# bjkomer/pyratslam

Measured on AMD Instinct MI355X. Metric: pose-cell steps/sec (64×64×36) + template-compares/sec at 1/2/4/8 GPU, higher is better.
Workload: dtype u8; 1 GPU; configs[1]: 64x64x36 pose-cell grid + 1000 stored 64x32 u8 templates per GPU; a step matches 10 batches of 1024 queries resident in HBM; templates_per_gpu=1000, templates_total=1000, queries_per_batch=1024, parallelism=library sharded over 1 GPU(s), none; pose cells replicated

## Files before the change

### pyratslam_amd/csrc/view_templates.hip

```cpp
#include <hip/hip_runtime.h>
#include <rccl/rccl.h>

#include <algorithm>
#include <climits>
#include <cstdint>
#include <cstdio>
#include <cstdlib>
#include <cstring>
#include <memory>
#include <vector>

#include "rs_common.h"
#include "vt_plan.h"

namespace {

constexpr int FAST_M = 8;
constexpr unsigned long long NO_KEY = ~0ull;

__device__ inline unsigned long long wave_min_u64(unsigned long long v) {
#pragma unroll
    for (int off = 32; off > 0; off >>= 1) {
        const unsigned long long o = __shfl_xor(v, off);
        v = o < v ? o : v;
// ... 821 lines not shown
                                       wave, cg, lane, failed, ids, tk, v0);
    if (threadIdx.x == 0 && tk.takes && failed == tk.last) *ctr = 0u;
    if constexpr (!MATRIX) {
        if (out.host) {
            __shared__ int s_last;
            asm volatile("s_waitcnt vmcnt(0)" ::: "memory");
            __syncthreads();
            if (threadIdx.x == 0) {
                __builtin_amdgcn_fence(__ATOMIC_RELEASE, "agent");
                s_last = __hip_atomic_fetch_add(out.done, 1u, __ATOMIC_RELAXED, __HIP_MEMORY_SCOPE_AGENT) ==
                         gridDim.x - 1;
                if (s_last) __builtin_amdgcn_fence(__ATOMIC_ACQUIRE, "agent");
            }
            __syncthreads();
            if (s_last) {
                for (int i = threadIdx.x; i < nq; i += blockDim.x) {
                    const unsigned long long k =
                        __hip_atomic_load(out.best + i, __ATOMIC_RELAXED, __HIP_MEMORY_SCOPE_AGENT);
                    __hip_atomic_store(out.best + i, ~0ull, __ATOMIC_RELAXED, __HIP_MEMORY_SCOPE_AGENT);
                    __hip_atomic_store(out.host + i, k, __ATOMIC_RELAXED, __HIP_MEMORY_SCOPE_SYSTEM);
                }
                if (threadIdx.x == 0) __hip_atomic_store(out.done, 0u, __ATOMIC_RELAXED, __HIP_MEMORY_SCOPE_AGENT);
            }
        }
    }
    VT_STAMP(6);
}

constexpr int PF_WAVES = 4;
#ifndef VT_PF_TPW
#define VT_PF_TPW (VT_PF_UNITS == 1 ? 8 / (VT_PF_CGS) : 1)
#endif
constexpr int PF_TPW = VT_PF_TPW;
#ifndef VT_PF_CPS
#define VT_PF_CPS (VT_PF_TPW >= 4 ? 1 : 2)
#endif
constexpr int PF_CPS = VT_PF_CPS;
#ifndef VT_PF_GRID_CAP
#define VT_PF_GRID_CAP 4096
#endif
constexpr int PF_NB = 4;
constexpr int PF_QW4 = PF_NU * PF_CGS * PL_NO * 2;
constexpr uint32_t PF_NONE = (1u << 26) - 1u;

__device__ __forceinline__ uint32_t wave_min_u32_dpp(uint32_t v) {
    v = min(v, (uint32_t)__builtin_amdgcn_update_dpp((int)v, (int)v, 0xB1, 0xF, 0xF, false));
    v = min(v, (uint32_t)__builtin_amdgcn_update_dpp((int)v, (int)v, 0x4E, 0xF, 0xF, false));
    v = min(v, (uint32_t)__builtin_amdgcn_update_dpp((int)v, (int)v, 0x141, 0xF, 0xF, false));
    v = min(v, (uint32_t)__builtin_amdgcn_update_dpp((int)v, (int)v, 0x140, 0xF, 0xF, false));
    return min(min((uint32_t)__builtin_amdgcn_readlane((int)v, 0), (uint32_t)__builtin_amdgcn_readlane((int)v, 16)),
               min((uint32_t)__builtin_amdgcn_readlane((int)v, 32), (uint32_t)__builtin_amdgcn_readlane((int)v, 48)));
}

__global__ __launch_bounds__(64 * PF_WAVES) __attribute__((amdgpu_waves_per_eu(4)))
void vt_prefilter_kernel(const uint4* __restrict__ planes, int ntb,
                                                                    int64_t count,
                                                                    const uint4* __restrict__ qc4,
                                                                    const uint32_t* __restrict__ qsj, int nq,
                                                                    uint32_t* __restrict__ minlb,
                                                                    uint32_t* __restrict__ second) {
    constexpr int M = FAST_M, NU = 64 / 4, S0 = M - 3;
    static_assert(PF_CGS % PF_CPS == 0 && PF_CGS >= 1 && PF_CGS <= PL_CG, "whole steps of column groups, of the unit");
    static_assert(PF_NU * PF_CGS * 32 * 255 < (int)PF_NONE, "a bound and a lane fit one word");
    __shared__ uint4 s_q[PF_NB][PF_NU][PF_CGS][PL_NO][2];
    __shared__ uint32_t s_qs[PF_NB][PF_NU][16];
    const int wave = __builtin_amdgcn_readfirstlane(threadIdx.x >> 6), lane = threadIdx.x & 63;
    const int tb0 = (blockIdx.x * PF_WAVES + wave) * PF_TPW;
    const bool live = tb0 < ntb;
    uint32_t P[PF_TPW][PF_NU][PF_CGS][8], ts[PF_TPW][PF_NU];
    bool valid[PF_TPW];
#pragma unroll
    for (int t = 0; t < PF_TPW; ++t) {
        const int tbc = min(tb0 + t, ntb - 1);
        valid[t] = tb0 + t < ntb && (int64_t)(tb0 + t) * 64 + lane < count;
#pragma unroll
        for (int u = 0; u < PF_NU; ++u) {
            ts[t][u] = 0u;
#pragma unroll
            for (int cg = 0; cg < PF_CGS; ++cg) {
                const uint4* src = planes + ((size_t)(tbc * PL_CG + cg) * NU + pf_unit(u)) * 128 + lane;
                const uint4 a = src[0], b = src[64];
                uint32_t(&p)[8] = P[t][u][cg];
                p[0] = a.x; p[1] = a.y; p[2] = a.z; p[3] = a.w;
                p[4] = b.x; p[5] = b.y; p[6] = b.z; p[7] = b.w;
#pragma unroll
                for (int k = 0; k < 8; ++k) ts[t][u] += (uint32_t)__builtin_popcount(p[k]) << k;
            }
        }
    }
    for (int q0 = blockIdx.y * PF_NB; q0 < nq; q0 += gridDim.y * PF_NB) {
        const int nb = min(PF_NB, nq - q0);
        __syncthreads();
        for (int i = threadIdx.x; i < nb * PF_QW4; i += blockDim.x) {
            const int qq = i / PF_QW4, r = i - qq * PF_QW4;
            const int u = r / (PF_CGS * PL_NO * 2), r2 = r - u * (PF_CGS * PL_NO * 2);
            const int cg = r2 / (PL_NO * 2), w = r2 - cg * (PL_NO * 2);
            (&s_q[0][0][0][0][0])[i] = qc_unit(qc4 + (size_t)(q0 + qq) * QC_Q4, cg,
                                               4 * pf_unit(u) - (M - 1) - S0 + (w >> 1), w & 1);
        }
        if ((int)threadIdx.x < nb * PF_NU * 16)
            (&s_qs[0][0][0])[threadIdx.x] = qsj[(size_t)q0 * PF_NU * 16 + threadIdx.x];
        __syncthreads();
        if (!live) continue;
#pragma unroll 1
        for (int qq = 0; qq < nb; ++qq) {
            uint32_t m[PF_TPW];
#pragma unroll
            for (int t = 0; t < PF_TPW; ++t) m[t] = 0xFFFFFFFFu;
            auto read_q = [&](int x, int u, int cp, uint32_t(&q)[PF_CPS][8]) {
#pragma unroll
                for (int i = 0; i < PF_CPS; ++i) {
                    const uint4 lo = s_q[qq][u][cp + i][PL_NO - 1 - x][0];
                    const uint4 hi = s_q[qq][u][cp + i][PL_NO - 1 - x][1];
                    q[i][0] = lo.x; q[i][1] = lo.y; q[i][2] = lo.z; q[i][3] = lo.w;
                    q[i][4] = hi.x; q[i][5] = hi.y; q[i][6] = hi.z; q[i][7] = hi.w;
                }
            };
#pragma unroll
            for (int x = 0; x < PL_NO; ++x) {
                uint32_t lb[PF_TPW];
#pragma unroll
                for (int t = 0; t < PF_TPW; ++t) lb[t] = 0u;
#pragma unroll
                for (int u = 0; u < PF_NU; ++u) {
                    uint32_t c[PF_TPW];
#pragma unroll
                    for (int t = 0; t < PF_TPW; ++t) c[t] = 0u;
#pragma unroll
                    for (int cp = 0; cp < PF_CGS; cp += PF_CPS) {
                        uint32_t q[PF_CPS][8], b[PF_TPW][PF_CPS];
                        read_q(x, u, cp, q);
#pragma unroll
                        for (int k = 0; k < 8; ++k)
#pragma unroll
                            for (int t = 0; t < PF_TPW; ++t)
#pragma unroll
                                for (int i = 0; i < PF_CPS; ++i)
                                    b[t][i] = __builtin_amdgcn_bitop3_b32(P[t][u][cp + i][k], q[i][k],
                                                                          k ? b[t][i] : 0u, 0x8E);
#pragma unroll
                        for (int t = 0; t < PF_TPW; ++t)
#pragma unroll
                            for (int i = 0; i < PF_CPS; ++i)
                                asm("v_bcnt_u32_b32 %0, %1, %2" : "=v"(c[t]) : "v"(b[t][i]), "v"(c[t]));
                        __builtin_amdgcn_sched_barrier(0);
                    }
                    const uint32_t qs = s_qs[qq][u][x];
#pragma unroll
                    for (int t = 0; t < PF_TPW; ++t)
                        lb[t] += (c[t] << 8) + (ts[t][u] - qs);
                }
#pragma unroll
                for (int t = 0; t < PF_TPW; ++t) m[t] = min(m[t], lb[t]);
            }
            uint32_t v[PF_TPW], w[PF_TPW];
#pragma unroll
            for (int t = 0; t < PF_TPW; ++t) {
                v[t] = wave_min_u32_dpp(valid[t] ? (m[t] << 6) | (uint32_t)lane : 0xFFFFFFFFu);
                w[t] = wave_min_u32_dpp(valid[t] && lane != (int)(v[t] & 63u) ? m[t] : PF_NONE);
            }
            if (lane == 0) {
#pragma unroll
                for (int t = 0; t < PF_TPW; ++t)
                    if (tb0 + t < ntb) {
                        minlb[(size_t)(tb0 + t) * nq + q0 + qq] = v[t] >> 6;
                        second[(size_t)(tb0 + t) * nq + q0 + qq] = (w[t] << 6) | (v[t] & 63u);
                    }
            }
        }
    }
}

constexpr int VT_LIST_T = 1024;
__device__ __forceinline__ void list_append(bool in, int q, unsigned* __restrict__ cnt, int* __restrict__ list) {
    __shared__ unsigned s_w[VT_LIST_T / 64];
    __shared__ unsigned s_base;
    const int lane = threadIdx.x & 63, wave = threadIdx.x >> 6;
    const unsigned long long mask = __ballot(in);
    if (lane == 0) s_w[wave] = (unsigned)__popcll(mask);
    __syncthreads();
    if (threadIdx.x == 0) {
        unsigned t = 0u;
        for (int w = 0; w < VT_LIST_T / 64; ++w) {
            const unsigned c = s_w[w];
            s_w[w] = t;
            t += c;
        }
        s_base = t ? atomicAdd(cnt, t) : 0u;
    }
    __syncthreads();
    if (in) list[s_base + s_w[wave] + (unsigned)__popcll(mask & ((1ull << lane) - 1ull))] = q;
}

constexpr int VT_VQ4 = PlaneLds<64>::QW / 4;
constexpr int VT_VR = QC_NA + 7;
__global__ __launch_bounds__(64) void vt_prune_verify_kernel(const uint32_t* __restrict__ minlb,
                                                             const uint32_t* __restrict__ second, int ntb, int nq,
                                                             const uint4* __restrict__ planes,
                                                             const uint32_t* __restrict__ tsum,
                                                             const uint4* __restrict__ qc4,
                                                             uint4* __restrict__ qp4,
                                                             const uint32_t* __restrict__ qsum,
                                                             unsigned long long* __restrict__ best, int rank,
                                                             int nranks, int* __restrict__ tbstar) {
    constexpr int M = FAST_M, NU = 64 / 4, NS = PlaneLds<64>::NS, S0 = M - 3, S1 = 64 - M - 1;
    static_assert(PL_NO * PL_CG <= 64, "one lane per (offset, column group)");
    constexpr int QK = (QC_Q4 + 63) / 64;
    __shared__ uint4 s_q[PL_CG * VT_VR * 2];
    __shared__ uint4 s_t[PL_CG * NU * 2];
    const int q = blockIdx.x, lane = threadIdx.x;
    const int x = lane >> 2, cg = lane & 3, o = x - (M - 1);
    uint4 qv[QK];
#pragma unroll
    for (int k = 0; k < QK; ++k) qv[k] = qc4[(size_t)q * QC_Q4 + min(lane + 64 * k, QC_Q4 - 1)];
    const uint32_t qs = qsum[q];
    unsigned long long pk = ~0ull;
    uint32_t sec = 0u, m2 = 0xFFFFFFFFu;
    for (int tb = lane; tb < ntb; tb += 64) {
        const unsigned long long k = ((unsigned long long)minlb[(size_t)tb * nq + q] << 32) | (unsigned)tb;
        const uint32_t s2 = second[(size_t)tb * nq + q];
        const bool lt = k < pk;
        m2 = min(m2, (uint32_t)((lt ? pk : k) >> 32));
        pk = lt ? k : pk;
        sec = lt ? s2 : sec;
    }
#pragma unroll
    for (int k = 0; k < QK; ++k) asm volatile("" : "+v"(qv[k].x), "+v"(qv[k].y), "+v"(qv[k].z), "+v"(qv[k].w));
    const unsigned long long mk = wave_min_u64(pk);
    const int tbs = (int)(unsigned)mk;
    uint32_t other = pk == mk ? m2 : (uint32_t)(pk >> 32);
#pragma unroll
    for (int off = 32; off > 0; off >>= 1) other = min(other, (uint32_t)__shfl_xor((int)other, off));
    sec = (uint32_t)__shfl((int)sec, __ffsll((unsigned long long)__ballot(pk == mk)) - 1);
    const int tl = (int)(sec & 63u);
    const uint32_t ts = x < PL_NO ? tsum[((size_t)tbs * 16 + x) * 64 + tl] : 0u;
    static_assert(PL_CG * NU * 2 == 128, "two template chunks per lane");
    const uint4 t0 = planes[((size_t)tbs * 128 + lane) * 64 + tl];
    const uint4 t1 = planes[((size_t)tbs * 128 + 64 + lane) * 64 + tl];
    s_t[lane] = t0;
    s_t[64 + lane] = t1;
#pragma unroll
    for (int k = 0; k < QK; ++k) {
        const int c = lane + 64 * k, g = c / (QC_NA * 2);
        if (c < QC_Q4) s_q[(g * VT_VR + 3) * 2 + (c - g * (QC_NA * 2))] = qv[k];
    }
    if (lane < 2 * PL_CG) s_q[((lane >> 1) * VT_VR + 3 + QC_NA) * 2 + (lane & 1)] = make_uint4(0u, 0u, 0u, 0u);
    __syncthreads();
    uint32_t cnt = 0u;
    if (x < PL_NO) {
        const int a = (-o - S0) >> 2;
        const uint32_t sh = 8u * (uint32_t)((-o - S0) & 3);
        const uint4* sq = s_q + (cg * VT_VR + 3 + a) * 2;
        uint4 la = sq[0], lc = sq[1];
#pragma unroll 4
        for (int j = 0; j < NU; ++j) {
            const bool in = 4 * j - o >= S0 && 4 * j - o <= S1;
            const uint4 ta = s_t[(cg * NU + j) * 2], tc = s_t[(cg * NU + j) * 2 + 1];
            const uint4 ha = sq[(j + 1) * 2], hc = sq[(j + 1) * 2 + 1];
            const uint4 qa = qc_shift(la, ha, sh), qc = qc_shift(lc, hc, sh);
            la = ha;
            lc = hc;
            uint32_t b = __builtin_amdgcn_bitop3_b32(ta.x, qa.x, 0u, 0x8E);
            b = __builtin_amdgcn_bitop3_b32(ta.y, qa.y, b, 0x8E);
            b = __builtin_amdgcn_bitop3_b32(ta.z, qa.z, b, 0x8E);
            b = __builtin_amdgcn_bitop3_b32(ta.w, qa.w, b, 0x8E);
            b = __builtin_amdgcn_bitop3_b32(tc.x, qc.x, b, 0x8E);
            b = __builtin_amdgcn_bitop3_b32(tc.y, qc.y, b, 0x8E);
            b = __builtin_amdgcn_bitop3_b32(tc.z, qc.z, b, 0x8E);
            b = __builtin_amdgcn_bitop3_b32(tc.w, qc.w, b, 0x8E);
            cnt += in ? (uint32_t)__builtin_popcount(b) : 0u;
        }
    }
    cnt += __shfl_xor(cnt, 1);
    cnt += __shfl_xor(cnt, 2);
    uint32_t u0 = x < PL_NO ? ts + 256u * cnt : 0xFFFFFFFFu;
#pragma unroll
    for (int off = 32; off > 0; off >>= 1) u0 = min(u0, (uint32_t)__shfl_xor(u0, off));
    u0 -= qs;
    const bool settled = (sec >> 6) > u0;
    if (!settled || other <= u0) {
#pragma unroll
        for (int k = 0; k < (VT_VQ4 + 63) / 64; ++k) {
            const int i = lane + 64 * k, g = i / (NS * 2), r = i - g * (NS * 2), si = r >> 1;
            if (i < VT_VQ4) {
                const uint4* su = s_q + (g * VT_VR + 3 + (si >> 2)) * 2 + (r & 1);
                qp4[(size_t)q * VT_VQ4 + i] = qc_shift(su[0], su[2], 8u * (uint32_t)(si & 3));
            }
        }
    }
    if (lane == 0) {
        if (settled) {
            const unsigned long long g = ((unsigned long long)tbs * 64 + tl) * nranks + rank;
            atomicMin(best + q, ((unsigned long long)u0 << 32) | g);
        }
        tbstar[q] = settled ? ~tbs : tbs;
    }
}

__global__ __launch_bounds__(VT_LIST_T) void vt_prune_first_kernel(int nq, const int* __restrict__ tbstar,
                                                                   unsigned* __restrict__ cnt,
                                                                   int* __restrict__ list,
                                                                   unsigned* __restrict__ verified,
                                                                   unsigned* __restrict__ cnt2, int ntb) {
    const int q = blockIdx.x * VT_LIST_T + threadIdx.x, tb = blockIdx.y;
    const int ts = q < nq ? tbstar[q] : INT_MAX;
    if (blockIdx.x == 0 && tb == 0)
        for (int b = threadIdx.x; b < ntb; b += VT_LIST_T) cnt2[b] = 0u;
    if (tb == 0) {
        const int n = __syncthreads_count(ts < 0);
        if (threadIdx.x == 0 && n) atomicAdd(verified, (unsigned)n);
    }
    list_append(ts == tb, q, cnt + tb, list + (size_t)tb * nq);
}

__global__ __launch_bounds__(VT_LIST_T) void vt_prune_rest_kernel(const uint32_t* __restrict__ minlb, int nq,
                                                                  const int* __restrict__ tbstar,
                                                                  const unsigned long long* __restrict__ best,
                                                                  unsigned* __restrict__ cnt,
                                                                  int* __restrict__ list,
                                                                  unsigned* __restrict__ cnt1,
                                                                  unsigned* __restrict__ verified, int ntb,
                                                                  unsigned long long* __restrict__ stat) {
    const int q = blockIdx.x * VT_LIST_T + threadIdx.x, tb = blockIdx.y;
    const int ts = q < nq ? tbstar[q] : 0;
    const bool in = q < nq && tb != (ts < 0 ? ~ts : ts) && minlb[(size_t)tb * nq + q] <= (uint32_t)(best[q] >> 32);
    list_append(in, q, cnt + tb, list + (size_t)tb * nq);
    if (blockIdx.x == 0 && tb == 0) {
        __shared__ unsigned long long s_sum;
        if (threadIdx.x == 0) s_sum = 0ull;
        __syncthreads();
        unsigned long long a = 0ull;
        for (int b = threadIdx.x; b < ntb; b += VT_LIST_T) {
            a += cnt1[b];
            cnt1[b] = 0u;
        }
        if (a) atomicAdd(&s_sum, a);
        __syncthreads();
        if (threadIdx.x == 0) {
            const unsigned v = *verified;
            *verified = 0u;
            stat[0] = s_sum + v;
            stat[2] = v;
        }
    }
}

template <typename T>
__device__ inline T sad_at(const T* __restrict__ a, const T* __restrict__ b, int W, int M, int o,
// ... 85 lines not shown
    int rank = 0, nranks = 1;
    ncclComm_t comm = nullptr;
    int64_t count = 0;
    int64_t localCap = 0;
    rs::DevBuf<uint4> dLib;
    hipStream_t stream = nullptr;
    int qCap = 0;
    rs::DevBuf<uint8_t> dQraw;
    rs::PinnedBuf<uint8_t> hQraw;
    bool qrawBusy = false;
    rs::DevBuf<uint2> dQf;
    rs::DevBuf<uint32_t> dQsum;
    rs::DevBuf<unsigned long long> dBest;
    rs::PinnedBuf<unsigned long long> hBest;
    bool stagingBusy = false;
    hipStream_t cstream = nullptr;
    hipEvent_t evScan = nullptr, evComm = nullptr;
    hipStream_t ustream = nullptr;
    hipEvent_t evUp[2] = {nullptr, nullptr}, evUsed[2] = {nullptr, nullptr};
    rs::DevBuf<uint8_t> dUp[2];
    size_t upCap = 0;
    rs::DevBuf<uint32_t> dQpStream;
    rs::DevBuf<uint32_t> dQsumStream;
    size_t qpStreamCap = 0;
    rs::DevBuf<unsigned long long> dStream;
    rs::PinnedBuf<unsigned long long> hStream;
    size_t streamCap = 0;
    bool streamClean = false;
    int bestClean = 0;
    int bestPending = 0;
    int idxCap = 0;
    rs::DevBuf<int32_t> dSrc;
    rs::DevBuf<int64_t> dDst;
    rs::PinnedBuf<int32_t> hSrc;
    rs::PinnedBuf<int64_t> hDst;
    int64_t candCap = 0;
    rs::DevBuf<uint4> dCand;
    size_t matCap = 0;
    rs::DevBuf<uint32_t> dMat;
    rs::PinnedBuf<uint32_t> hMat;
    hipEvent_t ev0 = nullptr, ev1 = nullptr;
    bool timing = false;
    bool timedScan = false;
    float lastMs = 0.f;
    int stagedQ = 0;
    bool planar = false;
    rs::DevBuf<uint32_t> dLibP, dLibTs, dCandP, dCandTs;
    rs::DevBuf<uint32_t> dQp, dQsumRaw;
    int planeSlots = 0;
    rs::DevBuf<unsigned> dCtr;
    rs::DevBuf<unsigned> dDone;
    bool keysFolded = false;
    int prune = 0;
    rs::DevBuf<uint32_t> dQsj;
    rs::DevBuf<uint32_t> dQsjStream;
    rs::DevBuf<uint32_t> dQc;
    rs::DevBuf<uint32_t> dQcStream;
    bool qpFull = true;
    bool qcValid = false;
    rs::DevBuf<uint32_t> dMinLB;
    rs::DevBuf<uint32_t> dSecond;
    rs::DevBuf<int> dList;
    size_t pruneCap = 0;
    rs::DevBuf<int> dTbStar;
    rs::DevBuf<unsigned> dListCnt;
    int listCntCap = 0;
    rs::DevBuf<unsigned long long> dPruneStat;
    int64_t prunePairs = 0;
    int prunePasses = 0;
    int pruneNtb = 0;
    rs::DevBuf<int32_t> dPix;
    int64_t frameBytes = 0;
    rs::DevBuf<uint8_t> dFrames;
    rs::PinnedBuf<uint8_t> hFrames;
    int frameCap = 0;
};

namespace {

size_t tblock_bytes(const rs_vt* h) { return (size_t)h->WD * h->HQ * 64 * 16; }
size_t pblock_bytes(const rs_vt* h) { return (size_t)PL_CG * (h->H / 4) * 128 * 16; }
constexpr size_t TS_BLOCK_BYTES = 16 * 64 * sizeof(uint32_t);
int plane_ns(const rs_vt* h) { return h->H - 2 * h->M + 3; }

template <class T>
int vt_realloc_blocks(rs_vt* h, rs::DevBuf<T>& buf, int64_t keep, int64_t blocks, size_t bb,
                      const char* what = "template buffer growth") {
    rs::DevBuf<T> nb;
    const size_t bytes = (size_t)blocks * bb;
    RS_TRY(nb.reserve(bytes / sizeof(T), what));
    RS_HIP(hipMemsetAsync(nb.get(), 0, bytes, h->stream));
    if (buf.get()) {
        if (keep > 0)
            RS_HIP(hipMemcpyAsync(nb.get(), buf.get(), (size_t)keep * bb, hipMemcpyDeviceToDevice, h->stream));
        RS_HIP(hipStreamSynchronize(h->stream));
    }
    buf = std::move(nb);
    return RS_OK;
}

int64_t local_count_of(const rs_vt* h, int64_t global_count) {
    return vt_plan::local_count_of(h->rank, h->nranks, global_count);
}

int vt_grow_lib(rs_vt* h, int64_t need_slots) {
    if (need_slots <= h->localCap) return RS_OK;
// ... 199 lines not shown
    const uint32_t* ts;
    int ntb;
    int64_t count;
    const QueryForms& q;
    int nq, nqc, rank, nranks;
};
template <int H, bool MATRIX, bool LIST>
void vt_launch_plane_scan(rs_vt* h, const PlaneScan& s, const ScanOut& out, const PlaneList& list) {
    hipLaunchKernelGGL((vt_scan_plane_kernel<H, MATRIX, LIST>), s.grid, dim3(64 * PL_CG * PL_SPLIT), 0, h->stream,
                       s.planes, s.ts, s.ntb, s.count, s.q.qp, s.q.qsum, s.nq, s.nqc, h->dCtr.get(), out, s.rank,
                       s.nranks, list);
}

int vt_ensure_prune_buffers(rs_vt* h, int ntb, int nq) {
    const size_t pairs = (size_t)ntb * nq;
    if (pairs > h->pruneCap) {
        const size_t cap = std::max(pairs, 2 * h->pruneCap);
        h->pruneCap = 0;
        RS_TRY(h->dMinLB.reserve(cap));
        RS_TRY(h->dSecond.reserve(cap));
        RS_TRY(h->dList.reserve(2 * cap));
        h->pruneCap = cap;
    }
    RS_TRY(h->dTbStar.reserve((size_t)nq));
    if (ntb > h->listCntCap) {
        const int cap = std::max(ntb, 2 * h->listCntCap);
        h->listCntCap = 0;
        RS_TRY(h->dListCnt.reserve(2 * (size_t)cap + 1));
        RS_HIP(hipMemsetAsync(h->dListCnt.get(), 0, sizeof(unsigned) * (2 * (size_t)cap + 1), h->stream));
        h->listCntCap = cap;
    }
    if (!h->dPruneStat.get()) {
        RS_TRY(h->dPruneStat.reserve(3));
        RS_HIP(hipMemsetAsync(h->dPruneStat.get(), 0, 3 * sizeof(unsigned long long), h->stream));
    }
    return RS_OK;
}

int vt_launch_pruned(rs_vt* h, const PlaneScan& s, const ScanOut& out) {
    const QueryForms& q = s.q;
    const int ntb = s.ntb, nq = s.nq;
    if (!h->qcValid) {
        hipLaunchKernelGGL(vt_qcompact_kernel, dim3((unsigned)nq), dim3(128), 0, h->stream,
                           reinterpret_cast<const uint4*>(q.qp), reinterpret_cast<uint4*>(q.qc));
        h->qcValid = true;
    }
    RS_TRY(vt_ensure_prune_buffers(h, ntb, nq));
    const size_t pairs = (size_t)ntb * nq;
    unsigned* cnt1 = h->dListCnt.get();
    unsigned* cnt2 = h->dListCnt.get() + h->listCntCap;
    unsigned* verified = h->dListCnt.get() + 2 * (size_t)h->listCntCap;
    int* list1 = h->dList.get();
    int* list2 = h->dList.get() + pairs;
    const vt_plan::Grid2 pf = vt_plan::prefilter_grid(ntb, nq, PF_WAVES * PF_TPW, PF_NB, VT_PF_GRID_CAP);
    hipLaunchKernelGGL(vt_prefilter_kernel, dim3((unsigned)pf.x, (unsigned)pf.y), dim3(64 * PF_WAVES), 0, h->stream,
                       s.planes, ntb, s.count, reinterpret_cast<const uint4*>(q.qc), q.qsj, nq, h->dMinLB.get(),
                       h->dSecond.get());
    hipLaunchKernelGGL(vt_prune_verify_kernel, dim3((unsigned)nq), dim3(64), 0, h->stream, h->dMinLB.get(),
                       h->dSecond.get(), ntb, nq, s.planes, s.ts, reinterpret_cast<const uint4*>(q.qc),
                       reinterpret_cast<uint4*>(q.qp), q.qsum, out.best, s.rank, s.nranks, h->dTbStar.get());
    const dim3 lgrid((unsigned)((nq + VT_LIST_T - 1) / VT_LIST_T), (unsigned)ntb);
    hipLaunchKernelGGL(vt_prune_first_kernel, lgrid, dim3(VT_LIST_T), 0, h->stream, nq, h->dTbStar.get(), cnt1,
                       list1, verified, cnt2, ntb);
    ScanOut po = out;
    po.host = nullptr;
    po.done = nullptr;
    vt_launch_plane_scan<64, false, true>(h, s, po, PlaneList{list1, cnt1, nq, VT_LIST_PER_B1});
    hipLaunchKernelGGL(vt_prune_rest_kernel, lgrid, dim3(VT_LIST_T), 0, h->stream, h->dMinLB.get(), nq,
                       h->dTbStar.get(), out.best, cnt2, list2, cnt1, verified, ntb, h->dPruneStat.get());
#ifdef VT_LIST_PER
    const int per2 = VT_LIST_PER;
#else
    const int per2 = vt_plan::list_per(ntb, h->planeSlots);
#endif
    vt_launch_plane_scan<64, false, true>(h, s, po, PlaneList{list2, cnt2, nq, per2});
    if (out.host) vt_launch_keys_export(h, out.best, nq, out.host, vt_plan::VT_EXPORT_BLOCKS);
    RS_HIP(hipGetLastError());
    h->prunePairs = (int64_t)pairs;
    h->prunePasses = 2;
    h->pruneNtb = ntb;
    return RS_OK;
}

template <bool MATRIX>
int vt_launch_plane(rs_vt* h, const QueryForms& q, bool cand, int64_t count, int nq, ScanOut out, int rank,
                    int nranks, int64_t tb0) {
    const int ntb = (int)((count + 63) / 64);
    const int nqc = vt_plan::plane_split(ntb, (nq + PL_NB - 1) / PL_NB, h->planeSlots, vt_nqc_env());
    if (8 * (size_t)ntb > h->dCtr.capacity()) {
        const size_t cap = std::max(8 * (size_t)ntb, 2 * h->dCtr.capacity());
        RS_TRY(h->dCtr.reserve(cap));
        RS_HIP(hipMemsetAsync(h->dCtr.get(), 0, sizeof(unsigned) * cap, h->stream));
    }
    RS_CHECK((int64_t)ntb * nqc < (1ll << 31), RS_ERR_ARG, "scan grid too large");
    const uint4* planes = reinterpret_cast<const uint4*>(
        reinterpret_cast<const uint8_t*>(cand ? h->dCandP.get() : h->dLibP.get()) + (size_t)tb0 * pblock_bytes(h));
    const uint32_t* ts = (cand ? h->dCandTs.get() : h->dLibTs.get()) + (size_t)tb0 * (TS_BLOCK_BYTES / 4);
    const PlaneScan s{dim3((unsigned)(ntb * nqc)), planes, ts, ntb, count, q, nq, nqc, rank, nranks};
    if constexpr (!MATRIX)
        if (vt_prunes(h, q, cand, tb0, count, nq)) return vt_launch_pruned(h, s, out);
    if (!h->qpFull) {
        hipLaunchKernelGGL(vt_qexpand_kernel, dim3((unsigned)nq), dim3(256), 0, h->stream,
                           reinterpret_cast<const uint4*>(q.qc), reinterpret_cast<uint4*>(q.qp));
        h->qpFull = true;
    }
    vt_by_h(h, [&](auto H) { vt_launch_plane_scan<decltype(H)::value, MATRIX, false>(h, s, out, PlaneList{}); });
    RS_HIP(hipGetLastError());
    return RS_OK;
}

template <bool MATRIX>
int vt_launch_scan(rs_vt* h, const QueryForms& q, bool cand, int64_t count, int nq, ScanOut out, int rank,
                   int nranks, int64_t tb0 = 0) {
// ... 331 lines not shown
    case vt_plan::StreamPath::HostGroups: RS_TRY(vt_stream_host_groups(h, nb, nq, queries, lc)); break;
    case vt_plan::StreamPath::PerBatch: RS_TRY(vt_stream_per_batch(h, nb, nq, queries, on_device, lc)); break;
    }
    vt_launch_keys_export(h, h->dStream.get(), (int)total, h->hStream.dev(), vt_plan::VT_EXPORT_BLOCKS_STREAM);
    RS_HIP(hipGetLastError());
    RS_HIP(hipStreamSynchronize(h->stream));
    h->streamClean = true;
    if (h->timedScan) RS_HIP(hipEventElapsedTime(&h->lastMs, h->ev0, h->ev1));
    vt_decode_keys(h->hStream.get(), total, best_score, best_index);
    return RS_OK;
}

int vt_match_impl(rs_vt* h, int nq, const uint8_t* queries, int mode, uint64_t* best_score,
                  int64_t* best_index, uint8_t* is_new, bool frames = false) {
    RS_CHECK(mode == RS_VT_FROZEN || mode == RS_VT_SEQUENTIAL, RS_ERR_ARG, "unknown mode %d", mode);
    RS_TRY(vt_scan_local_impl(h, nq, queries, frames, h->nranks == 1));
    if (nq == 0) return RS_OK;
    RS_TRY(vt_fetch_keys(h, nq, true));
    return vt_resolve_impl(h, nq, h->hBest.get(), mode, best_score, best_index, is_new);
}

}

extern "C" {

int rs_vt_create(int H, int W, int max_offset, uint64_t thr, int64_t capacity, int device,
                 rs_vt** out) {
    rs::clear_error();
    RS_CHECK(out, RS_ERR_ARG, "null output handle pointer");
    *out = nullptr;
    RS_CHECK(H > 0 && W > 0 && H <= 4096 && W <= 4096, RS_ERR_ARG, "bad template shape (%d, %d)", H, W);
    RS_CHECK(max_offset >= 1 && max_offset <= 64, RS_ERR_ARG, "max_offset %d outside [1, 64]", max_offset);
    RS_CHECK(capacity >= 0, RS_ERR_ARG, "negative capacity");
    RS_CHECK((uint64_t)H * W * 255u < 0xFFFFFFFFull, RS_ERR_ARG, "template too large");
    int ndev = 0;
    RS_HIP(hipGetDeviceCount(&ndev));
    RS_CHECK(device >= 0 && device < ndev, RS_ERR_ARG, "device %d not in [0, %d)", device, ndev);
    RS_HIP(hipSetDevice(device));
    std::unique_ptr<rs_vt, int (*)(rs_vt*)> owner(new rs_vt(), rs_vt_destroy);
    rs_vt* const h = owner.get();
    h->H = H; h->W = W; h->M = max_offset; h->thr = (double)thr; h->device = device;
    h->WD = (W + 3) / 4;
    h->HQ = (H + 3) / 4;
    h->planar = W == 8 * PL_CG && (H == 64 || H == 32) && max_offset == FAST_M;
    if (const char* e = std::getenv("RS_VT_SCAN")) {
        if (std::strcmp(e, "carry") == 0) h->planar = false;
        else RS_CHECK(std::strcmp(e, "plane") == 0 || e[0] == 0, RS_ERR_ARG, "RS_VT_SCAN='%s': expected plane or carry", e);
    }
    if (h->planar && h->H == 64) {
        const char* e = std::getenv("RS_VT_PRUNE");
        if (!e || e[0] == 0 || std::strcmp(e, "1") == 0) h->prune = 1;
        else if (std::strcmp(e, "force") == 0) h->prune = 2;
        else RS_CHECK(std::strcmp(e, "0") == 0, RS_ERR_ARG, "RS_VT_PRUNE='%s': expected 0, 1 or force", e);
    }
    if (h->planar) {
        int per_cu = 0, cus = 0;
        hipFuncAttributes fa{};
        const void* fn = vt_by_h(h, [](auto H) {
            return reinterpret_cast<const void*>(vt_scan_plane_kernel<decltype(H)::value, false>);
        });
        hipError_t oe = hipOccupancyMaxActiveBlocksPerMultiprocessor(&per_cu, fn, 64 * PL_CG * PL_SPLIT, 0);
        if (oe == hipSuccess) oe = hipFuncGetAttributes(&fa, fn);
        if (oe == hipSuccess) oe = hipDeviceGetAttribute(&cus, hipDeviceAttributeMultiprocessorCount, device);
        RS_CHECK(oe == hipSuccess, RS_ERR_HIP, "occupancy query failed: %s", hipGetErrorString(oe));
        const int vg = std::max(8, (fa.numRegs + 7) / 8 * 8);
        const int by_vgpr = (512 / vg) * 4 / (PL_CG * PL_SPLIT);
        const int by_lds = fa.sharedSizeBytes > 0 ? (int)(160 * 1024 / fa.sharedSizeBytes) : per_cu;
        const int api = per_cu;
        per_cu = std::max(1, std::min({api, by_vgpr, by_lds}));
        h->planeSlots = std::max(1, per_cu * cus);
    }
    hipError_t e = hipStreamCreateWithFlags(&h->stream, hipStreamNonBlocking);
    if (e == hipSuccess) e = hipEventCreate(&h->ev0);
    if (e == hipSuccess) e = hipEventCreate(&h->ev1);
    RS_CHECK(e == hipSuccess, RS_ERR_HIP, "stream/event creation failed: %s", hipGetErrorString(e));
    RS_TRY(vt_grow_lib(h, capacity > 0 ? capacity : 64));
    RS_TRY(vt_grow_queries(h, 64));
    RS_TRY(vt_grow_index(h, 64));
    *out = owner.release();
    return RS_OK;
}

int rs_vt_destroy(rs_vt* h) {
    if (!h) return RS_OK;
    (void)hipSetDevice(h->device);
    hipError_t se = hipSuccess;
    for (hipStream_t st : {h->stream, h->cstream, h->ustream})
        if (st) {
            const hipError_t e = hipStreamSynchronize(st);
            if (se == hipSuccess) se = e;
        }
    if (h->comm) (void)ncclCommDestroy(h->comm);
    if (h->ev0) (void)hipEventDestroy(h->ev0);
    if (h->ev1) (void)hipEventDestroy(h->ev1);
    if (h->evScan) (void)hipEventDestroy(h->evScan);
    if (h->evComm) (void)hipEventDestroy(h->evComm);
    if (h->cstream) (void)hipStreamDestroy(h->cstream);
    for (int i = 0; i < 2; ++i) {
        if (h->evUp[i]) (void)hipEventDestroy(h->evUp[i]);
        if (h->evUsed[i]) (void)hipEventDestroy(h->evUsed[i]);
    }
    if (h->ustream) (void)hipStreamDestroy(h->ustream);
    if (h->stream) (void)hipStreamDestroy(h->stream);
    delete h;
    RS_CHECK(se == hipSuccess, RS_ERR_HIP, "work queued before rs_vt_destroy failed: %s", hipGetErrorString(se));
    return RS_OK;
// ... 338 lines not shown
```

### pyratslam_amd/csrc/vt_plan.h

```cpp
#pragma once

#include <algorithm>
#include <cstdint>

namespace vt_plan {

inline int64_t local_count_of(int rank, int nranks, int64_t global_count) {
    if (global_count <= rank) return 0;
    return (global_count - rank + nranks - 1) / nranks;
}

inline int plane_split(int ntb, int nbatch, int slots, int nqc_override) {
    int nqc = nqc_override;
    if (nqc_override <= 0) {
        const int fill = (slots + ntb - 1) / ntb;
        nqc = std::max(32, std::min(4 * fill, std::max(128, fill)));
    }
    nqc = std::min(nqc, std::max(1, nbatch));
    if (nqc >= 8) nqc &= ~7;
    return nqc;
}

#if defined(__HIPCC__)
#define VT_PLAN_HD __host__ __device__
#else
#define VT_PLAN_HD
#endif
struct Take {
    int nbatch;
    int nstat;
    int sb;
    int ndyn;
    bool takes;
    unsigned last;
};
VT_PLAN_HD inline int take_groups(int nblk) { return nblk >= 8 ? 8 : 1; }
VT_PLAN_HD inline int take_group_of(int l, int nblk) { return nblk >= 8 ? (l & 7) : 0; }
VT_PLAN_HD inline int list_use(int nq, int nb, int per, int nqc) {
    const int use = ((nq + nb - 1) / nb + per - 1) / per;
    if (nqc >= 8) {
        const int u8 = (use + 7) & ~7;
        return u8 < 8 ? 8 : (u8 > nqc ? nqc : u8);
    }
    return use < 1 ? 1 : (use > nqc ? nqc : use);
}
inline int list_per(int ntb, int resident_blocks) { return ntb < resident_blocks ? 4 : 3; }
VT_PLAN_HD inline Take take_plan(int nq, int nb, int l, int nblk) {
    const int G = take_groups(nblk), g = take_group_of(l, nblk);
    Take t;
    t.nbatch = ((nq + nb - 1) / nb - g + G - 1) / G;
    t.nstat = nblk / G;
    t.sb = G == 8 ? (l >> 3) : l;
    t.ndyn = t.nbatch > t.nstat ? t.nbatch - t.nstat : 0;
    t.takes = t.ndyn > 0 && t.sb < t.nbatch;
    t.last = (unsigned)(t.ndyn + (t.nstat < t.nbatch ? t.nstat : t.nbatch) - 1);
    return t;
}
VT_PLAN_HD inline int take_batch(const Take& t, unsigned take) { return t.nstat + (int)take; }

constexpr int VT_PRUNE_MIN_Q = 512;
constexpr int64_t VT_PRUNE_MAX_TB = 65535;

inline bool prunes(int H, bool cand, int64_t tb0, bool forms, int64_t ntb, int prune, int nq) {
    return H == 64 && !cand && tb0 == 0 && forms && ntb <= VT_PRUNE_MAX_TB &&
           (prune == 2 || (prune == 1 && nq >= VT_PRUNE_MIN_Q && ntb >= 2));
}

struct Grid2 {
    int x, y;
};
inline Grid2 prefilter_grid(int ntb, int nq, int tb_per_block, int q_per_batch, int cap) {
    const int nqb = (nq + q_per_batch - 1) / q_per_batch, pfx = (ntb + tb_per_block - 1) / tb_per_block;
    return {pfx, std::min(nqb, std::max(1, cap / pfx))};
}

constexpr int VT_EXPORT_BLOCKS = 64, VT_EXPORT_BLOCKS_STREAM = 256;
inline int export_grid(int64_t n, int max_blocks) { return (int)std::min<int64_t>((n + 255) / 256, max_blocks); }

constexpr int VT_ZC_MAX = 64;
inline bool stages_in_place(bool planar, int nq, bool zc_on) { return planar && nq <= VT_ZC_MAX && zc_on; }

constexpr int VT_POLL_MAX = 4096;
inline bool polls_keys(bool poll_on, bool timed, int nq) { return poll_on && !timed && nq <= VT_POLL_MAX; }
inline bool folds_keys(bool fold_ok, bool planar, int64_t local_count, bool poll_on, bool timing, int nq) {
    return fold_ok && planar && local_count > 0 && polls_keys(poll_on, timing, nq);
}

enum class StreamPath { Fused, HostGroups, PerBatch };
inline StreamPath stream_path(bool on_device, bool planar, int nb) {
    if (!planar) return StreamPath::PerBatch;
    if (!on_device) return StreamPath::HostGroups;
    return nb > 1 ? StreamPath::Fused : StreamPath::PerBatch;
}

constexpr int VT_UP_GROUP = 16;
struct HostGroup {
    int b0, n;
    int buf;
    bool waits;
};
struct HostGroups {
    int gb;
    int first;
    int nb;
    HostGroup group(int g) const {
        const int b0 = g == 0 ? 0 : std::min(nb, first + (g - 1) * gb);
        return {b0, std::min(g == 0 ? first : gb, nb - b0), g & 1, g >= 2};
    }
};
inline HostGroups host_groups(int nb) {
    const int gb = std::min(nb, std::max(2, std::min(VT_UP_GROUP, (nb - 1) / 3)));
    return {gb, nb >= 4 ? 1 : gb, nb};
}

}
```

Baseline: 28.08 billion compares/s.

## Fuse prefilter and prune-verify into one front kernel for small template sets

Adds a fused front kernel that runs the lower-bound prefilter and then the per-query verification in the same block. It keeps each wave's pick state in shared memory, so the separate prune-verify launch and the global `second` buffer round trip go away. It is chosen by default when all template blocks fit in one block's chunk, and an env var can force it on or off. The prefilter also folds the template and query sums into biased constants, replacing a per-unit subtraction with one add. The cost is a larger shared-memory footprint and a grid of one block column, which may lower occupancy.

```diff
diff --git a/pyratslam_amd/csrc/view_templates.hip b/pyratslam_amd/csrc/view_templates.hip
--- a/pyratslam_amd/csrc/view_templates.hip
+++ b/pyratslam_amd/csrc/view_templates.hip
@@ -897,6 +897,109 @@
                min((uint32_t)__builtin_amdgcn_readlane((int)v, 32), (uint32_t)__builtin_amdgcn_readlane((int)v, 48)));
 }
 
+constexpr uint32_t PF_BIAS = PF_CGS * 32 * 256;
+static_assert(PF_NU * (PF_CGS * 32 * 256 + PF_BIAS) < (1u << 31), "the biased bounds do not wrap");
+
+__device__ __forceinline__ void pf_load(const uint4* __restrict__ planes, int ntb, int64_t count, int tb0, int lane,
+                                        uint32_t (&P)[PF_TPW][PF_NU][PF_CGS][8], uint32_t (&tsb)[PF_TPW],
+                                        bool (&valid)[PF_TPW]) {
+    constexpr int NU = 64 / 4;
+#pragma unroll
+    for (int t = 0; t < PF_TPW; ++t) {
+        const int tbc = min(tb0 + t, ntb - 1);
+        valid[t] = tb0 + t < ntb && (int64_t)(tb0 + t) * 64 + lane < count;
+        tsb[t] = 0u - PF_NU * PF_BIAS;
+#pragma unroll
+        for (int u = 0; u < PF_NU; ++u) {
+#pragma unroll
+            for (int cg = 0; cg < PF_CGS; ++cg) {
+                const uint4* src = planes + ((size_t)(tbc * PL_CG + cg) * NU + pf_unit(u)) * 128 + lane;
+                const uint4 a = src[0], b = src[64];
+                uint32_t(&p)[8] = P[t][u][cg];
+                p[0] = a.x; p[1] = a.y; p[2] = a.z; p[3] = a.w;
+                p[4] = b.x; p[5] = b.y; p[6] = b.z; p[7] = b.w;
+#pragma unroll
+                for (int k = 0; k < 8; ++k) tsb[t] += (uint32_t)__builtin_popcount(p[k]) << k;
+            }
+        }
+    }
+}
+
+__device__ __forceinline__ void pf_stage(const uint4* __restrict__ qc4, const uint32_t* __restrict__ qsj, int q0, int nb,
+                                         uint4 (&s_q)[PF_NB][PF_NU][PF_CGS][PL_NO][2],
+                                         uint32_t (&s_qs)[PF_NB][PF_NU][16]) {
+    constexpr int M = FAST_M, S0 = M - 3;
+    for (int i = threadIdx.x; i < nb * PF_QW4; i += blockDim.x) {
+        const int qq = i / PF_QW4, r = i - qq * PF_QW4;
+        const int u = r / (PF_CGS * PL_NO * 2), r2 = r - u * (PF_CGS * PL_NO * 2);
+        const int cg = r2 / (PL_NO * 2), w = r2 - cg * (PL_NO * 2);
+        (&s_q[0][0][0][0][0])[i] = qc_unit(qc4 + (size_t)(q0 + qq) * QC_Q4, cg,
+                                           4 * pf_unit(u) - (M - 1) - S0 + (w >> 1), w & 1);
+    }
+    if ((int)threadIdx.x < nb * PF_NU * 16)
+        (&s_qs[0][0][0])[threadIdx.x] = PF_BIAS - qsj[(size_t)q0 * PF_NU * 16 + threadIdx.x];
+}
+
+__device__ __forceinline__ void pf_walk(const uint32_t (&P)[PF_TPW][PF_NU][PF_CGS][8], const uint32_t (&tsb)[PF_TPW],
+                                        const bool (&valid)[PF_TPW], const uint4 (&sq)[PF_NU][PF_CGS][PL_NO][2],
+                                        const uint32_t (&sqs)[PF_NU][16], int lane, uint32_t (&v)[PF_TPW],
+                                        uint32_t (&w)[PF_TPW]) {
+    uint32_t m[PF_TPW];
+#pragma unroll
+    for (int t = 0; t < PF_TPW; ++t) m[t] = 0xFFFFFFFFu;
+    auto read_q = [&](int x, int u, int cp, uint32_t(&q)[PF_CPS][8]) {
+#pragma unroll
+        for (int i = 0; i < PF_CPS; ++i) {
+            const uint4 lo = sq[u][cp + i][PL_NO - 1 - x][0];
+            const uint4 hi = sq[u][cp + i][PL_NO - 1 - x][1];
+            q[i][0] = lo.x; q[i][1] = lo.y; q[i][2] = lo.z; q[i][3] = lo.w;
+            q[i][4] = hi.x; q[i][5] = hi.y; q[i][6] = hi.z; q[i][7] = hi.w;
+        }
+    };
+#pragma unroll
+    for (int x = 0; x < PL_NO; ++x) {
+        uint32_t lb[PF_TPW];
+#pragma unroll
+        for (int t = 0; t < PF_TPW; ++t) lb[t] = 0u;
+#pragma unroll
+        for (int u = 0; u < PF_NU; ++u) {
+            uint32_t c[PF_TPW];
+#pragma unroll
+            for (int t = 0; t < PF_TPW; ++t) c[t] = 0u;
+#pragma unroll
+            for (int cp = 0; cp < PF_CGS; cp += PF_CPS) {
+                uint32_t q[PF_CPS][8], b[PF_TPW][PF_CPS];
+                read_q(x, u, cp, q);
+#pragma unroll
+                for (int k = 0; k < 8; ++k)
+#pragma unroll
+                    for (int t = 0; t < PF_TPW; ++t)
+#pragma unroll
+                        for (int i = 0; i < PF_CPS; ++i)
+                            b[t][i] = __builtin_amdgcn_bitop3_b32(P[t][u][cp + i][k], q[i][k],
+                                                                  k ? b[t][i] : 0u, 0x8E);
+#pragma unroll
+                for (int t = 0; t < PF_TPW; ++t)
+#pragma unroll
+                    for (int i = 0; i < PF_CPS; ++i)
+                        asm("v_bcnt_u32_b32 %0, %1, %2" : "=v"(c[t]) : "v"(b[t][i]), "v"(c[t]));
+                __builtin_amdgcn_sched_barrier(0);
+            }
+            const uint32_t qsb = sqs[u][x];
+#pragma unroll
+            for (int t = 0; t < PF_TPW; ++t) lb[t] += (c[t] << 8) + qsb;
+        }
+#pragma unroll
+        for (int t = 0; t < PF_TPW; ++t) m[t] = min(m[t], lb[t]);
+    }
+#pragma unroll
+    for (int t = 0; t < PF_TPW; ++t) {
+        const uint32_t lbt = m[t] + tsb[t];
+        v[t] = wave_min_u32_dpp(valid[t] ? (lbt << 6) | (uint32_t)lane : 0xFFFFFFFFu);
+        w[t] = wave_min_u32_dpp(valid[t] && lane != (int)(v[t] & 63u) ? lbt : PF_NONE);
+    }
+}
+
 __global__ __launch_bounds__(64 * PF_WAVES) __attribute__((amdgpu_waves_per_eu(4)))
 void vt_prefilter_kernel(const uint4* __restrict__ planes, int ntb,
                                                                     int64_t count,
@@ -904,7 +1007,6 @@
                                                                     const uint32_t* __restrict__ qsj, int nq,
                                                                     uint32_t* __restrict__ minlb,
                                                                     uint32_t* __restrict__ second) {
-    constexpr int M = FAST_M, NU = 64 / 4, S0 = M - 3;
     static_assert(PF_CGS % PF_CPS == 0 && PF_CGS >= 1 && PF_CGS <= PL_CG, "whole steps of column groups, of the unit");
     static_assert(PF_NU * PF_CGS * 32 * 255 < (int)PF_NONE, "a bound and a lane fit one word");
     __shared__ uint4 s_q[PF_NB][PF_NU][PF_CGS][PL_NO][2];
@@ -912,98 +1014,19 @@
     const int wave = __builtin_amdgcn_readfirstlane(threadIdx.x >> 6), lane = threadIdx.x & 63;
     const int tb0 = (blockIdx.x * PF_WAVES + wave) * PF_TPW;
     const bool live = tb0 < ntb;
-    uint32_t P[PF_TPW][PF_NU][PF_CGS][8], ts[PF_TPW][PF_NU];
+    uint32_t P[PF_TPW][PF_NU][PF_CGS][8], tsb[PF_TPW];
     bool valid[PF_TPW];
-#pragma unroll
-    for (int t = 0; t < PF_TPW; ++t) {
-        const int tbc = min(tb0 + t, ntb - 1);
-        valid[t] = tb0 + t < ntb && (int64_t)(tb0 + t) * 64 + lane < count;
-#pragma unroll
-        for (int u = 0; u < PF_NU; ++u) {
-            ts[t][u] = 0u;
-#pragma unroll
-            for (int cg = 0; cg < PF_CGS; ++cg) {
-                const uint4* src = planes + ((size_t)(tbc * PL_CG + cg) * NU + pf_unit(u)) * 128 + lane;
-                const uint4 a = src[0], b = src[64];
-                uint32_t(&p)[8] = P[t][u][cg];
-                p[0] = a.x; p[1] = a.y; p[2] = a.z; p[3] = a.w;
-                p[4] = b.x; p[5] = b.y; p[6] = b.z; p[7] = b.w;
-#pragma unroll
-                for (int k = 0; k < 8; ++k) ts[t][u] += (uint32_t)__builtin_popcount(p[k]) << k;
-            }
-        }
-    }
+    pf_load(planes, ntb, count, tb0, lane, P, tsb, valid);
     for (int q0 = blockIdx.y * PF_NB; q0 < nq; q0 += gridDim.y * PF_NB) {
         const int nb = min(PF_NB, nq - q0);
         __syncthreads();
-        for (int i = threadIdx.x; i < nb * PF_QW4; i += blockDim.x) {
-            const int qq = i / PF_QW4, r = i - qq * PF_QW4;
-            const int u = r / (PF_CGS * PL_NO * 2), r2 = r - u * (PF_CGS * PL_NO * 2);
-            const int cg = r2 / (PL_NO * 2), w = r2 - cg * (PL_NO * 2);
-            (&s_q[0][0][0][0][0])[i] = qc_unit(qc4 + (size_t)(q0 + qq) * QC_Q4, cg,
-                                               4 * pf_unit(u) - (M - 1) - S0 + (w >> 1), w & 1);
-        }
-        if ((int)threadIdx.x < nb * PF_NU * 16)
-            (&s_qs[0][0][0])[threadIdx.x] = qsj[(size_t)q0 * PF_NU * 16 + threadIdx.x];
+        pf_stage(qc4, qsj, q0, nb, s_q, s_qs);
         __syncthreads();
         if (!live) continue;
 #pragma unroll 1
         for (int qq = 0; qq < nb; ++qq) {
-            uint32_t m[PF_TPW];
-#pragma unroll
-            for (int t = 0; t < PF_TPW; ++t) m[t] = 0xFFFFFFFFu;
-            auto read_q = [&](int x, int u, int cp, uint32_t(&q)[PF_CPS][8]) {
-#pragma unroll
-                for (int i = 0; i < PF_CPS; ++i) {
-                    const uint4 lo = s_q[qq][u][cp + i][PL_NO - 1 - x][0];
-                    const uint4 hi = s_q[qq][u][cp + i][PL_NO - 1 - x][1];
-                    q[i][0] = lo.x; q[i][1] = lo.y; q[i][2] = lo.z; q[i][3] = lo.w;
-                    q[i][4] = hi.x; q[i][5] = hi.y; q[i][6] = hi.z; q[i][7] = hi.w;
-                }
-            };
-#pragma unroll
-            for (int x = 0; x < PL_NO; ++x) {
-                uint32_t lb[PF_TPW];
-#pragma unroll
-                for (int t = 0; t < PF_TPW; ++t) lb[t] = 0u;
-#pragma unroll
-                for (int u = 0; u < PF_NU; ++u) {
-                    uint32_t c[PF_TPW];
-#pragma unroll
-                    for (int t = 0; t < PF_TPW; ++t) c[t] = 0u;
-#pragma unroll
-                    for (int cp = 0; cp < PF_CGS; cp += PF_CPS) {
-                        uint32_t q[PF_CPS][8], b[PF_TPW][PF_CPS];
-                        read_q(x, u, cp, q);
-#pragma unroll
-                        for (int k = 0; k < 8; ++k)
-#pragma unroll
-                            for (int t = 0; t < PF_TPW; ++t)
-#pragma unroll
-                                for (int i = 0; i < PF_CPS; ++i)
-                                    b[t][i] = __builtin_amdgcn_bitop3_b32(P[t][u][cp + i][k], q[i][k],
-                                                                          k ? b[t][i] : 0u, 0x8E);
-#pragma unroll
-                        for (int t = 0; t < PF_TPW; ++t)
-#pragma unroll
-                            for (int i = 0; i < PF_CPS; ++i)
-                                asm("v_bcnt_u32_b32 %0, %1, %2" : "=v"(c[t]) : "v"(b[t][i]), "v"(c[t]));
-                        __builtin_amdgcn_sched_barrier(0);
-                    }
-                    const uint32_t qs = s_qs[qq][u][x];
-#pragma unroll
-                    for (int t = 0; t < PF_TPW; ++t)
-                        lb[t] += (c[t] << 8) + (ts[t][u] - qs);
-                }
-#pragma unroll
-                for (int t = 0; t < PF_TPW; ++t) m[t] = min(m[t], lb[t]);
-            }
             uint32_t v[PF_TPW], w[PF_TPW];
-#pragma unroll
-            for (int t = 0; t < PF_TPW; ++t) {
-                v[t] = wave_min_u32_dpp(valid[t] ? (m[t] << 6) | (uint32_t)lane : 0xFFFFFFFFu);
-                w[t] = wave_min_u32_dpp(valid[t] && lane != (int)(v[t] & 63u) ? m[t] : PF_NONE);
-            }
+            pf_walk(P, tsb, valid, s_q[qq], s_qs[qq], lane, v, w);
             if (lane == 0) {
 #pragma unroll
                 for (int t = 0; t < PF_TPW; ++t)
@@ -1039,21 +1062,18 @@
 
 constexpr int VT_VQ4 = PlaneLds<64>::QW / 4;
 constexpr int VT_VR = QC_NA + 7;
-__global__ __launch_bounds__(64) void vt_prune_verify_kernel(const uint32_t* __restrict__ minlb,
-                                                             const uint32_t* __restrict__ second, int ntb, int nq,
-                                                             const uint4* __restrict__ planes,
-                                                             const uint32_t* __restrict__ tsum,
-                                                             const uint4* __restrict__ qc4,
-                                                             uint4* __restrict__ qp4,
-                                                             const uint32_t* __restrict__ qsum,
-                                                             unsigned long long* __restrict__ best, int rank,
-                                                             int nranks, int* __restrict__ tbstar) {
+constexpr int VT_VQS = PL_CG * VT_VR * 2, VT_VTS = PL_CG * (64 / 4) * 2;
+template <class Pick>
+__device__ __forceinline__ void vt_verify_query(int q, bool act, int lane, Pick&& pick, int nq,
+                                                const uint4* __restrict__ planes,
+                                                const uint32_t* __restrict__ tsum,
+                                                const uint4* __restrict__ qc4, uint4* __restrict__ qp4,
+                                                const uint32_t* __restrict__ qsum,
+                                                unsigned long long* __restrict__ best, int rank, int nranks,
+                                                int* __restrict__ tbstar, uint4* s_q, uint4* s_t) {
     constexpr int M = FAST_M, NU = 64 / 4, NS = PlaneLds<64>::NS, S0 = M - 3, S1 = 64 - M - 1;
     static_assert(PL_NO * PL_CG <= 64, "one lane per (offset, column group)");
     constexpr int QK = (QC_Q4 + 63) / 64;
-    __shared__ uint4 s_q[PL_CG * VT_VR * 2];
-    __shared__ uint4 s_t[PL_CG * NU * 2];
-    const int q = blockIdx.x, lane = threadIdx.x;
     const int x = lane >> 2, cg = lane & 3, o = x - (M - 1);
     uint4 qv[QK];
 #pragma unroll
@@ -1061,14 +1081,7 @@
     const uint32_t qs = qsum[q];
     unsigned long long pk = ~0ull;
     uint32_t sec = 0u, m2 = 0xFFFFFFFFu;
-    for (int tb = lane; tb < ntb; tb += 64) {
-        const unsigned long long k = ((unsigned long long)minlb[(size_t)tb * nq + q] << 32) | (unsigned)tb;
-        const uint32_t s2 = second[(size_t)tb * nq + q];
-        const bool lt = k < pk;
-        m2 = min(m2, (uint32_t)((lt ? pk : k) >> 32));
-        pk = lt ? k : pk;
-        sec = lt ? s2 : sec;
-    }
+    pick(pk, sec, m2);
 #pragma unroll
     for (int k = 0; k < QK; ++k) asm volatile("" : "+v"(qv[k].x), "+v"(qv[k].y), "+v"(qv[k].z), "+v"(qv[k].w));
     const unsigned long long mk = wave_min_u64(pk);
@@ -1123,7 +1136,7 @@
     for (int off = 32; off > 0; off >>= 1) u0 = min(u0, (uint32_t)__shfl_xor(u0, off));
     u0 -= qs;
     const bool settled = (sec >> 6) > u0;
-    if (!settled || other <= u0) {
+    if (act && (!settled || other <= u0)) {
 #pragma unroll
         for (int k = 0; k < (VT_VQ4 + 63) / 64; ++k) {
             const int i = lane + 64 * k, g = i / (NS * 2), r = i - g * (NS * 2), si = r >> 1;
@@ -1133,12 +1146,101 @@
             }
         }
     }
-    if (lane == 0) {
+    if (act && lane == 0) {
         if (settled) {
             const unsigned long long g = ((unsigned long long)tbs * 64 + tl) * nranks + rank;
             atomicMin(best + q, ((unsigned long long)u0 << 32) | g);
         }
         tbstar[q] = settled ? ~tbs : tbs;
+    }
+}
+
+__global__ __launch_bounds__(64) void vt_prune_verify_kernel(const uint32_t* __restrict__ minlb,
+                                                             const uint32_t* __restrict__ second, int ntb, int nq,
+                                                             const uint4* __restrict__ planes,
+                                                             const uint32_t* __restrict__ tsum,
+                                                             const uint4* __restrict__ qc4,
+                                                             uint4* __restrict__ qp4,
+                                                             const uint32_t* __restrict__ qsum,
+                                                             unsigned long long* __restrict__ best, int rank,
+                                                             int nranks, int* __restrict__ tbstar) {
+    __shared__ uint4 s_q[VT_VQS];
+    __shared__ uint4 s_t[VT_VTS];
+    const int q = blockIdx.x, lane = threadIdx.x;
+    vt_verify_query(q, true, lane, [&](unsigned long long& pk, uint32_t& sec, uint32_t& m2) {
+        for (int tb = lane; tb < ntb; tb += 64) {
+            const unsigned long long k = ((unsigned long long)minlb[(size_t)tb * nq + q] << 32) | (unsigned)tb;
+            const uint32_t s2 = second[(size_t)tb * nq + q];
+            const bool lt = k < pk;
+            m2 = min(m2, (uint32_t)((lt ? pk : k) >> 32));
+            pk = lt ? k : pk;
+            sec = lt ? s2 : sec;
+        }
+    }, nq, planes, tsum, qc4, qp4, qsum, best, rank, nranks, tbstar, s_q, s_t);
+}
+
+__global__ __launch_bounds__(64 * PF_WAVES) __attribute__((amdgpu_waves_per_eu(4)))
+void vt_front_kernel(const uint4* __restrict__ planes, int ntb, int64_t count, const uint4* __restrict__ qc4,
+                     const uint32_t* __restrict__ qsj, int nq, uint32_t* __restrict__ minlb,
+                     const uint32_t* __restrict__ tsum, uint4* __restrict__ qp4,
+                     const uint32_t* __restrict__ qsum, unsigned long long* __restrict__ best, int rank,
+                     int nranks, int* __restrict__ tbstar) {
+    constexpr int CH = PF_WAVES * PF_TPW;
+    static_assert(PF_WAVES == PF_NB, "one wave per query of the group in the tail");
+    static_assert(CH <= 64, "one lane per block of a chunk");
+    __shared__ uint4 s_q[PF_NB][PF_NU][PF_CGS][PL_NO][2];
+    __shared__ uint32_t s_qs[PF_NB][PF_NU][16];
+    __shared__ uint2 s_pick[2][PF_NB][CH];
+    __shared__ uint4 s_vq[PF_WAVES][VT_VQS];
+    __shared__ uint4 s_vt[PF_WAVES][VT_VTS];
+    const int wave = __builtin_amdgcn_readfirstlane(threadIdx.x >> 6), lane = threadIdx.x & 63;
+    int par = 0;
+    for (int q0 = blockIdx.y * PF_NB; q0 < nq; q0 += gridDim.y * PF_NB) {
+        const int nb = min(PF_NB, nq - q0);
+        const int qw = min(wave, nb - 1);
+        __syncthreads();
+        pf_stage(qc4, qsj, q0, nb, s_q, s_qs);
+        __syncthreads();
+        unsigned long long pk = ~0ull;
+        uint32_t sec = 0u, m2 = 0xFFFFFFFFu;
+        for (int c0 = 0; c0 < ntb; c0 += CH) {
+            const int tb0 = c0 + wave * PF_TPW;
+            if (tb0 < ntb) {
+                uint32_t P[PF_TPW][PF_NU][PF_CGS][8], tsb[PF_TPW];
+                bool valid[PF_TPW];
+                pf_load(planes, ntb, count, tb0, lane, P, tsb, valid);
+#pragma unroll 1
+                for (int qq = 0; qq < nb; ++qq) {
+                    uint32_t v[PF_TPW], w[PF_TPW];
+                    pf_walk(P, tsb, valid, s_q[qq], s_qs[qq], lane, v, w);
+                    if (lane == 0) {
+#pragma unroll
+                        for (int t = 0; t < PF_TPW; ++t)
+                            if (tb0 + t < ntb) {
+                                minlb[(size_t)(tb0 + t) * nq + q0 + qq] = v[t] >> 6;
+                                s_pick[par][qq][wave * PF_TPW + t] = make_uint2(v[t] >> 6, (w[t] << 6) | (v[t] & 63u));
+                            }
+                    }
+                }
+            }
+            __syncthreads();
+            if (lane < CH && c0 + lane < ntb) {
+                const uint2 e = s_pick[par][qw][lane];
+                const unsigned long long k = ((unsigned long long)e.x << 32) | (unsigned)(c0 + lane);
+                const bool lt = k < pk;
+                m2 = min(m2, (uint32_t)((lt ? pk : k) >> 32));
+                pk = lt ? k : pk;
+                sec = lt ? e.y : sec;
+            }
+            par ^= 1;
+        }
+        int vl = lane;
+        asm volatile("" : "+v"(vl));
+        vt_verify_query(q0 + qw, wave < nb, vl, [&](unsigned long long& pk_, uint32_t& sec_, uint32_t& m2_) {
+            pk_ = pk;
+            sec_ = sec;
+            m2_ = m2;
+        }, nq, planes, tsum, qc4, qp4, qsum, best, rank, nranks, tbstar, s_vq[wave], s_vt[wave]);
     }
 }
 
@@ -1330,6 +1432,7 @@
     rs::DevBuf<unsigned> dDone;
     bool keysFolded = false;
     int prune = 0;
+    int front = 1;
     rs::DevBuf<uint32_t> dQsj;
     rs::DevBuf<uint32_t> dQsjStream;
     rs::DevBuf<uint32_t> dQc;
@@ -1635,13 +1738,21 @@
     unsigned* verified = h->dListCnt.get() + 2 * (size_t)h->listCntCap;
     int* list1 = h->dList.get();
     int* list2 = h->dList.get() + pairs;
-    const vt_plan::Grid2 pf = vt_plan::prefilter_grid(ntb, nq, PF_WAVES * PF_TPW, PF_NB, VT_PF_GRID_CAP);
-    hipLaunchKernelGGL(vt_prefilter_kernel, dim3((unsigned)pf.x, (unsigned)pf.y), dim3(64 * PF_WAVES), 0, h->stream,
-                       s.planes, ntb, s.count, reinterpret_cast<const uint4*>(q.qc), q.qsj, nq, h->dMinLB.get(),
-                       h->dSecond.get());
-    hipLaunchKernelGGL(vt_prune_verify_kernel, dim3((unsigned)nq), dim3(64), 0, h->stream, h->dMinLB.get(),
-                       h->dSecond.get(), ntb, nq, s.planes, s.ts, reinterpret_cast<const uint4*>(q.qc),
-                       reinterpret_cast<uint4*>(q.qp), q.qsum, out.best, s.rank, s.nranks, h->dTbStar.get());
+    if (h->front == 2 || (h->front == 1 && vt_plan::front_fused(ntb, PF_WAVES * PF_TPW))) {
+        const vt_plan::Grid2 fg = vt_plan::front_grid(nq, PF_NB, VT_PF_GRID_CAP);
+        hipLaunchKernelGGL(vt_front_kernel, dim3((unsigned)fg.x, (unsigned)fg.y), dim3(64 * PF_WAVES), 0, h->stream,
+                           s.planes, ntb, s.count, reinterpret_cast<const uint4*>(q.qc), q.qsj, nq, h->dMinLB.get(),
+                           s.ts, reinterpret_cast<uint4*>(q.qp), q.qsum, out.best, s.rank, s.nranks,
+                           h->dTbStar.get());
+    } else {
+        const vt_plan::Grid2 pf = vt_plan::prefilter_grid(ntb, nq, PF_WAVES * PF_TPW, PF_NB, VT_PF_GRID_CAP);
+        hipLaunchKernelGGL(vt_prefilter_kernel, dim3((unsigned)pf.x, (unsigned)pf.y), dim3(64 * PF_WAVES), 0,
+                           h->stream, s.planes, ntb, s.count, reinterpret_cast<const uint4*>(q.qc), q.qsj, nq,
+                           h->dMinLB.get(), h->dSecond.get());
+        hipLaunchKernelGGL(vt_prune_verify_kernel, dim3((unsigned)nq), dim3(64), 0, h->stream, h->dMinLB.get(),
+                           h->dSecond.get(), ntb, nq, s.planes, s.ts, reinterpret_cast<const uint4*>(q.qc),
+                           reinterpret_cast<uint4*>(q.qp), q.qsum, out.best, s.rank, s.nranks, h->dTbStar.get());
+    }
     const dim3 lgrid((unsigned)((nq + VT_LIST_T - 1) / VT_LIST_T), (unsigned)ntb);
     hipLaunchKernelGGL(vt_prune_first_kernel, lgrid, dim3(VT_LIST_T), 0, h->stream, nq, h->dTbStar.get(), cnt1,
                        list1, verified, cnt2, ntb);
@@ -2079,6 +2190,15 @@
         if (!e || e[0] == 0 || std::strcmp(e, "1") == 0) h->prune = 1;
         else if (std::strcmp(e, "force") == 0) h->prune = 2;
         else RS_CHECK(std::strcmp(e, "0") == 0, RS_ERR_ARG, "RS_VT_PRUNE='%s': expected 0, 1 or force", e);
+    }
+    if (h->planar && h->H == 64) {
+        const char* e = std::getenv("RS_VT_FRONT");
+        if (!e || e[0] == 0 || std::strcmp(e, "1") == 0) h->front = 1;
+        else if (std::strcmp(e, "force") == 0) h->front = 2;
+        else {
+            RS_CHECK(std::strcmp(e, "0") == 0, RS_ERR_ARG, "RS_VT_FRONT='%s': expected 0, 1 or force", e);
+            h->front = 0;
+        }
     }
     if (h->planar) {
         int per_cu = 0, cus = 0;
diff --git a/pyratslam_amd/csrc/vt_plan.h b/pyratslam_amd/csrc/vt_plan.h
--- a/pyratslam_amd/csrc/vt_plan.h
+++ b/pyratslam_amd/csrc/vt_plan.h
@@ -74,6 +74,11 @@
     return {pfx, std::min(nqb, std::max(1, cap / pfx))};
 }
 
+inline bool front_fused(int ntb, int tb_per_block) { return ntb <= tb_per_block; }
+inline Grid2 front_grid(int nq, int q_per_batch, int cap) {
+    return {1, std::max(1, std::min((nq + q_per_batch - 1) / q_per_batch, cap))};
+}
+
 constexpr int VT_EXPORT_BLOCKS = 64, VT_EXPORT_BLOCKS_STREAM = 256;
 inline int export_grid(int64_t n, int max_blocks) { return (int)std::min<int64_t>((n + 255) / 256, max_blocks); }
 
```

New measurement: 28.75 billion compares/s (median of 6 runs). 1.02x the previous value.
